# CasperTheCat/Vermilion

Measured on AMD Instinct MI355X. Metric: Mrays/sec (primary+secondary), 1920x1080 Sponza, higher is better.
Workload: dtype f32

## Files before the change

include/vermilion_hip.h:

```cpp
#ifndef VERMILION_HIP_H
#define VERMILION_HIP_H

#include <stdint.h>

#ifdef __cplusplus
extern "C" {
#endif

#define VMX_ABI_VERSION 2

#define VMX_OK 0
#define VMX_ERR_INVALID 1
#define VMX_ERR_NO_DEVICE 2
#define VMX_ERR_HIP 3
#define VMX_ERR_DEPTH 4
#define VMX_ERR_NOMEM 5

#define VMX_SPHERE_EMIT 1u

#define VMX_SAMPLING_PARITY 0u
#define VMX_SAMPLING_CORRECTED 1u
#define VMX_SAMPLING_MODE_MASK 0xFFu
#define VMX_SAMPLING_LIBM_DOUBLE 0x100u
#define VMX_SAMPLING_ELIDE_DEAD 0x200u
// ... 146 lines not shown
int vmx_query_device(const vmx_scene *scene, uint32_t mode, const void *d_origin, const void *d_dir,
                     const void *d_tmax, uint32_t n, void *d_tri_id, void *d_t, void *d_hit, void *stream);
int vmx_query(const vmx_scene *scene, uint32_t mode, const float *origin, const float *dir, const float *tmax,
              uint32_t n, int32_t *tri_id, float *t, uint8_t *hit);
int vmx_raycast_device(const vmx_scene *scene, const void *d_origin, const void *d_dir, uint32_t n, void *d_out,
                       uint32_t flags, void *stream);
int vmx_raycast_camera_device(const vmx_scene *scene, const vmx_camera *cam, const vmx_opts *opts, uint32_t k,
                              void *d_out, uint32_t flags, void *stream);

int vmx_primary_ids(const vmx_scene *scene, const vmx_camera *cam, const vmx_opts *opts, uint32_t k,
                    int32_t *tri_id, float *t);

int vmx_pixel_claims(const vmx_scene *scene, const vmx_camera *cam, const vmx_opts *opts, uint32_t *claims_out,
                     uint32_t *n_claimed);
int vmx_fused_camera_paths(const vmx_scene *scene, uint64_t *paths);
int vmx_pixel_claim_lists(const vmx_scene *scene, const vmx_camera *cam, const vmx_opts *opts, uint32_t *claims_out,
                          uint32_t *lists_out, uint32_t *n_claimed);
int vmx_list_settled_rays(const vmx_scene *scene, uint64_t *rays);
int vmx_guide_rays(const vmx_scene *scene, uint64_t *settled, uint64_t *fallback);
int vmx_guide_list_entries(const vmx_scene *scene, uint64_t *entries);
int vmx_guide_fused_rays(const vmx_scene *scene, uint64_t *settled, uint64_t *fallback);
int vmx_guide_trace(const vmx_scene *scene, const float *origin, const float *dir, uint32_t n, const vmx_opts *opts,
                    uint32_t flags, uint32_t grid_blocks, uint8_t *settled, uint32_t *slot, float *t);
int vmx_guide_trace_visits(const vmx_scene *scene, const float *origin, const float *dir, uint32_t n, const vmx_opts *opts,
                           uint32_t flags, uint32_t grid_blocks, uint8_t *settled, uint32_t *slot, float *t,
                           uint32_t *inner_visits, uint32_t *tri_tests);
int vmx_radiance(const vmx_scene *scene, const float *origin, const float *dir, uint32_t n,
                 const vmx_opts *opts, float *out, vmx_stats *stats);

int vmx_trig(const float *x, uint32_t n, float *cos_out, float *sin_out, int device);
// ... 252 lines not shown
```

vermilion_amd/_lib.py:

```python
import ctypes as C
import os

_HERE = os.path.dirname(os.path.abspath(__file__))
LIB_PATH = os.environ.get("VMX_LIB") or os.path.join(_HERE, "libvermilion_hip.so")

VMX_OK = 0
VMX_ERR_INVALID = 1
VMX_ERR_NO_DEVICE = 2
VMX_ERR_HIP = 3
VMX_ERR_DEPTH = 4
VMX_ERR_NOMEM = 5

VMX_SPHERE_EMIT = 1
VMX_SAMPLING_PARITY = 0
VMX_SAMPLING_CORRECTED = 1
VMX_SAMPLING_LIBM_DOUBLE = 0x100
VMX_SAMPLING_ELIDE_DEAD = 0x200
VMX_BVH_REFERENCE = 0
VMX_BVH_SAH = 1
VMX_BVH_LBVH = 2
VMX_BVH_PLOC = 3
VMX_BF_ABS_INT = 1
VMX_ROTATION_DEGREES = 0
VMX_ROTATION_RADIANS = 1
# ... 274 lines not shown
    "vmx_scene_compute_units": (C.c_uint32, [_P]),
    "vmx_scene_bvh": (C.c_int, [_P, _P, _P, _P, _P, _P]),
    "vmx_scene_update": (C.c_int, [_P, _P, _P, _P, C.c_uint32, C.c_uint32]),
    "vmx_scene_update_device": (C.c_int, [_P, _P, _P, _P, C.c_uint32, C.c_uint32, _P]),
    "vmx_scene_set_spheres": (C.c_int, [_P, _P, C.c_uint32]),
    "vmx_trace": (C.c_int, [_P, _P, _P, C.c_uint32, _P, _P]),
    "vmx_raycast": (C.c_int, [_P, _P, _P, C.c_uint32, _P]),
    "vmx_query_device": (C.c_int, [_P, C.c_uint32, _P, _P, _P, C.c_uint32, _P, _P, _P, _P]),
    "vmx_query": (C.c_int, [_P, C.c_uint32, _P, _P, _P, C.c_uint32, _P, _P, _P]),
    "vmx_raycast_device": (C.c_int, [_P, _P, _P, C.c_uint32, _P, C.c_uint32, _P]),
    "vmx_raycast_camera_device": (C.c_int, [_P, C.POINTER(CameraDesc), C.POINTER(Opts), C.c_uint32, _P, C.c_uint32,
                                            _P]),
    "vmx_primary_ids": (C.c_int, [_P, C.POINTER(CameraDesc), C.POINTER(Opts), C.c_uint32, _P, _P]),
    "vmx_pixel_claims": (C.c_int, [_P, C.POINTER(CameraDesc), C.POINTER(Opts), _P, C.POINTER(C.c_uint32)]),
    "vmx_fused_camera_paths": (C.c_int, [_P, C.POINTER(C.c_uint64)]),
    "vmx_pixel_claim_lists": (C.c_int, [_P, C.POINTER(CameraDesc), C.POINTER(Opts), _P, _P, C.POINTER(C.c_uint32)]),
    "vmx_list_settled_rays": (C.c_int, [_P, C.POINTER(C.c_uint64)]),
    "vmx_guide_rays": (C.c_int, [_P, C.POINTER(C.c_uint64), C.POINTER(C.c_uint64)]),
    "vmx_guide_list_entries": (C.c_int, [_P, C.POINTER(C.c_uint64)]),
    "vmx_guide_fused_rays": (C.c_int, [_P, C.POINTER(C.c_uint64), C.POINTER(C.c_uint64)]),
    "vmx_guide_trace": (C.c_int, [_P, _P, _P, C.c_uint32, _P, C.c_uint32, C.c_uint32, _P, _P, _P]),
    "vmx_guide_trace_visits": (C.c_int, [_P, _P, _P, C.c_uint32, _P, C.c_uint32, C.c_uint32, _P, _P, _P, _P, _P]),
    "vmx_radiance": (C.c_int, [_P, _P, _P, C.c_uint32, C.POINTER(Opts), _P, C.POINTER(Stats)]),
    "vmx_trig": (C.c_int, [_P, C.c_uint32, _P, _P, C.c_int]),
    "vmx_local_rows": (C.c_int, [C.c_uint32, C.c_uint32, C.c_uint32, C.c_uint32, C.POINTER(C.c_uint32)]),
    "vmx_render": (C.c_int, [_P, C.POINTER(CameraDesc), C.POINTER(Opts), _P, C.POINTER(Stats)]),
    "vmx_render_device": (C.c_int, [_P, C.POINTER(CameraDesc), C.POINTER(Opts), _P, _P, C.POINTER(Stats)]),
    "vmx_progressive_begin": (C.c_int, [_P, C.POINTER(CameraDesc), C.POINTER(Opts), _P, C.POINTER(_P)]),
    "vmx_progressive_step": (C.c_int, [_P, C.c_uint32, C.POINTER(Stats)]),
    "vmx_progressive_info_get": (C.c_int, [_P, C.POINTER(ProgressiveInfo)]),
# ... 125 lines not shown
```

vermilion_amd/csrc/api_claims.inc:

```
namespace {

constexpr uint32_t kClaimMinSamples = 64;
uint32_t claim_min_samples() {
#ifdef VMX_AB_KERNELS
    if (const char *e = std::getenv("VMX_CLAIM_MIN_SPP")) {
        const unsigned long v = std::strtoul(e, nullptr, 10);
        if (v) return (uint32_t)std::min<unsigned long>(v, 0xFFFFFFFFul);
    }
#endif
    return kClaimMinSamples;
}

int build_claims(vmx_scene *sc, const FrameDev &fr, const Tuning &tn, uint32_t npix, bool lists, hipStream_t s) {
    Workspace &ws = sc->ws;
    if (ws.claims.ensure((size_t)npix + 2)) return fail(VMX_ERR_NOMEM, "hipMalloc failed for the pixel claims");
    if (lists && ws.claim_lists.ensure((size_t)npix * kListWords)) return fail(VMX_ERR_NOMEM, "hipMalloc failed for the claim lists");
    WorkDev wk = make_work(nullptr, nullptr);
    wk.cam_inner = ws.cam_inner.p, wk.cam_tris = ws.cam_inner.p + std::max<size_t>(sc->n_inner, 1) * 64 * 8;
    const uint64_t tiles = (uint64_t)((fr.width + 7u) / 8u) * ((fr.local_rows + 7u) / 8u);
    if (tiles * 64 > 0xFFFFFFFFull) return fail(VMX_ERR_INVALID, "frame too large for the pixel claims");
    int cblocks = 0;
    HIP_TRY((hipError_t)query_pixel_claims_blocks_per_cu(kPathsBlock, (kPathsBlock / 64) * (tn.lds_primary + 1) * 512, &cblocks));
    if (cblocks < 1) return fail(VMX_ERR_HIP, "kernel does not fit on a CU (LDS stack too deep?)");
    LaunchCfg cfg = paths_cfg(sc, tn.lds_primary, tiles * 64, cblocks);
// ... 70 lines not shown
    vmx_scene *sc = const_cast<vmx_scene *>(csc);
    if (!sc || !rays) return fail(VMX_ERR_INVALID, "NULL argument");
    std::lock_guard<std::mutex> lock(sc->mu);
    *rays = sc->list_settled;
    return VMX_OK;
}

int vmx_fused_camera_paths(const vmx_scene *csc, uint64_t *paths) {
    vmx_scene *sc = const_cast<vmx_scene *>(csc);
    if (!sc || !paths) return fail(VMX_ERR_INVALID, "NULL argument");
    std::lock_guard<std::mutex> lock(sc->mu);
    *paths = sc->fused_paths;
    return VMX_OK;
}

}
```

vermilion_amd/csrc/api_render.inc:

```
namespace {

int nee_launch_cfg(vmx_scene *sc, hipStream_t s, const Tuning &tn, uint64_t items, bool rays, WorkDev &wk, LaunchCfg &cfg,
                   bool budgeted = false);

Tuning make_tuning(const vmx_scene *sc, const vmx_opts *o) {
    Tuning tn;
    tn.refill_min = o->reserved[3] ? o->reserved[3] : 8u;
    tn.refill_primary = o->reserved[3] ? o->reserved[3] : 64u;
    tn.shade_min = o->reserved[4] ? o->reserved[4] : 16u;
    tn.leaf_min = 0xFFFFFFFFu;
    tn.sort_mode = o->reserved[5];
    const uint32_t cap = o->reserved[6];
    tn.lds_entries = std::min(sc->dev.stack_entries, cap ? cap : 10u);
    tn.lds_primary = std::min(sc->dev.stack_entries, cap ? cap : (uint32_t)VMX_LDS_PRIMARY);
    tn.lds_bounce = std::min(sc->dev.stack_entries, cap ? cap : 9u);
    tn.tail_threshold = o->reserved[2] ? o->reserved[2] : (16u << 20);
    return tn;
}


int bind_stack(vmx_scene *sc, const Tuning &tn, uint32_t entries, uint32_t grid, uint64_t items, WorkDev &wk, bool guided) {
    const uint64_t per_lane = items / ((uint64_t)grid * kPathsBlock);
    wk.reserve = per_lane >= 256 ? 256u : (per_lane >= 64 ? 128u : 64u);
    wk.lds_entries = entries;
// ... 137 lines not shown
    DevCounters h;
    HIP_TRY(hipMemcpy(&h, ws.counters.p, sizeof(h), hipMemcpyDeviceToHost));
    if (h.overflow) return fail(VMX_ERR_NOMEM, "path queue overflow (sub-queues full); lower max paths per pass");
    vmx_stats local_stats;
    if (!stats) stats = &local_stats;
    std::memset(stats, 0, sizeof(*stats));
    stage_out(stats->primary, h.stage[0]);
    stage_out(stats->bounce, h.stage[1]);
    stats->rays_primary = h.stage[0].rays;
    stats->rays_secondary = h.stage[1].rays;
    stats->samples = h.samples;
    stats->samples_discarded = h.discarded;
    stats->passes = passes;
    stats->kernel_launches = launches;
    sc->fused_paths = h.fused;
    sc->list_settled = h.listed;
    unsigned long long guide_rays[2] = {0, 0};
    if (ws.guide_ctr.p) HIP_TRY(hipMemcpy(guide_rays, ws.guide_ctr.p, sizeof(guide_rays), hipMemcpyDeviceToHost));
    sc->guide_settled = guide_rays[0], sc->guide_fallback = guide_rays[1];
    unsigned long long fused_rays[2] = {0, 0};
    if (ws.guide_fused_ctr.p) HIP_TRY(hipMemcpy(fused_rays, ws.guide_fused_ctr.p, sizeof(fused_rays), hipMemcpyDeviceToHost));
    sc->guide_fused_settled = fused_rays[0], sc->guide_fused_fallback = fused_rays[1];
    sc->guide_entries = ws.guide_entries, ws.guide_entries = 0;
    std::memset(&sc->timings, 0, sizeof(sc->timings));
    for (auto &tl : timed) {
        float ms = 0.f;
        HIP_TRY(hipEventElapsedTime(&ms, tl.a, tl.b));
        if (tl.stage >= 0) {
            vmx_stage_stats &st = tl.stage == 0 ? stats->primary : (tl.stage == 1 ? stats->bounce : stats->shade);
            st.ms += ms;
// ... 15 lines not shown
    const uint32_t bits = opts->reserved[0];
    Forms f;
    f.pipeline = bits & kFormPipeline;
    f.count = opts->collect_counters != 0;
    f.split_any = f.pipeline == 0 || f.pipeline == 4;
    f.legacy = f.pipeline >= 2 && f.pipeline <= 3;
    f.two_phase = !f.count && !(bits & kFormOnePhase) && fr.r2scale == 10.0f;
    f.sorted = f.two_phase && !(bits & kFormKeepEnds);
    f.pool = ab_pool_bit(opts) && !f.sorted && !f.count;
    f.guide = sc->guide.valid && !f.count && !ab_pool_bit(opts) && !(bits & kFormNoGuide);
    f.bounce_records = f.split_any && !f.two_phase && !f.count && !f.pool && fr.r2scale == 10.0f;
    f.elide = f.split_any && fr.elide_dead;
    f.claims_on = f.split_any && !f.count && !f.elide && !(bits & kFormNoClaims);
    f.fuse_on = f.claims_on && !f.two_phase && !f.sorted && !(bits & kFormNoFuse);
    f.lists_on = f.claims_on && !(bits & kFormNoLists);
    return f;
}

int render_setup(vmx_scene *sc, const vmx_camera *cam, const vmx_opts *opts, PixelBufs *pixels, float *d_out, hipStream_t s,
                 RenderJob &job) {
    FrameDev &fr = job.fr;
    int rc = make_frame(*cam, *opts, fr);
    if (rc) return rc;
    job.opts = *opts;
    job.pixels = pixels, job.d_out = d_out, job.s = s;
    Workspace &ws = sc->ws;
    const uint32_t W = fr.width, rows = fr.local_rows;
    const uint32_t npix = job.npix = W * rows;
    if (opts->collect_counters) fr.elide_dead = 0;
    if ((opts->reserved[0] & kFormPipeline) > 4 || (opts->reserved[0] & ~kFormsRender)) return fail(VMX_ERR_INVALID, "unknown pipeline form");
// ... 300 lines not shown
    } else {
        LAUNCH_TRY(launch_shade(sc->dev, fr, wk, job.px, job.pa, qi[0], 0, ws.counters.p, false, (uint32_t)sc->num_cus, s));
    }
    return timed_end(job.timed, s);
}

int pass_split(vmx_scene *sc, RenderJob &job, WorkDev &wk) {
    Workspace &ws = sc->ws;
    const Tuning &tn = job.tn;
    hipStream_t s = job.s;
    const uint64_t items = (uint64_t)wk.n_pad * wk.samples;
    wk.refill_min = tn.refill_primary;
    wk.cam_inner = ws.cam_inner.p, wk.cam_tris = ws.cam_inner.p + std::max<size_t>(sc->n_inner, 1) * 64 * 8;
    wk.cam_n_inner = sc->n_inner;
    wk.claims = job.claims;
    wk.claim_lists = job.f.elide ? nullptr : job.claim_lists, wk.list_ctr = ws.counters.p;
    LaunchCfg cfg = paths_cfg(sc, tn.lds_primary, items, job.tb);
    int rc = bind_stack(sc, tn, tn.lds_primary, cfg.grid, items, wk);
    if (rc) return rc;
    HIP_TRY(hipMemsetAsync(ws.heads.p, 0, kSubQueues * 32 * 4, s));
    SplitRoute r;
    if ((rc = split_raygen(sc, job, wk, r))) return rc;
    if ((rc = split_trace(sc, job, wk, r, cfg))) return rc;
    if ((rc = split_shade(sc, job, wk, r))) return rc;
    job.launches += 4;
    return run_ids(sc, job.fr, job.pa, job.qi, 0, ws.counters.p, job.f, tn, s, job.timed, job.launches, job.tbb, job.rb);
}

int render_pass(vmx_scene *sc, RenderJob &job, uint32_t cap, uint32_t *taken) {
    Workspace &ws = sc->ws;
// ... 124 lines not shown
```

vermilion_amd/csrc/vmx_device.h:

```cpp
#pragma once
#include <stdint.h>

namespace vmx {

constexpr uint32_t kLeafBit = 0x80000000u;
constexpr uint32_t kLeafStartMask = 0x03FFFFFFu;
constexpr uint32_t kLeafCountShift = 26;
constexpr uint32_t kMaxLeafSize = 31;
constexpr uint32_t kMaxTris = kLeafStartMask + 1;
constexpr uint32_t kMaxSpheres = 16;
constexpr uint32_t kMaxStack = 64;

struct InnerRecord {
    float lmin[3];
    float lmax[3];
    float rmin[3];
    float rmax[3];
    uint32_t left, right, pad0, pad1;
};
static_assert(sizeof(InnerRecord) == 64, "inner record must be 64 bytes");

struct TriRecord {
    float v0[3];
    float e1[3];
// ... 32 lines not shown
    uint32_t tex_w, tex_h, tex_c;
    uint32_t tri_off;
    const float *tex1;
    uint32_t tex1_w, tex1_h, tex1_c;
    uint32_t emit_prefix;
};

struct StageCounters {
    unsigned long long rays, inner_visits, tri_tests, tri_hits, continued;
};
struct DevCounters {
    StageCounters stage[2];
    unsigned long long samples, discarded, pixels_done, overflow;
    unsigned long long fused;
    unsigned long long listed;
};

struct FastDiv {
    uint32_t m, sh1, sh2, d;
};
inline FastDiv make_fastdiv(uint32_t d) {
    if (d == 0) d = 1;
    uint32_t l = 0;
    while ((1ull << l) < d) ++l;
    FastDiv f;
    f.m = (uint32_t)((((1ull << l) - d) << 32) / d + 1ull);
    f.sh1 = l < 1 ? l : 1u;
    f.sh2 = l > 0 ? l - 1 : 0u;
    f.d = d;
    return f;
// ... 29 lines not shown
```

vermilion_amd/csrc/vmx_host.h:

```cpp
namespace {

thread_local std::string g_err;

int fail(int code, const std::string &msg) {
    g_err = msg;
    return code;
}

#define HIP_TRY(expr)                                                                              \
    do {                                                                                           \
        hipError_t e_ = (expr);                                                                    \
        if (e_ != hipSuccess)                                                                      \
            return fail(VMX_ERR_HIP, std::string(#expr) + ": " + hipGetErrorString(e_));           \
    } while (0)

#define LAUNCH_TRY(expr)                                                                           \
    do {                                                                                           \
        int e_ = (expr);                                                                           \
        if (e_ != 0)                                                                               \
            return fail(VMX_ERR_HIP, std::string(#expr) + ": " + hipGetErrorString((hipError_t)e_)); \
    } while (0)

const vmx_sphere kReferenceSpheres[8] = {
    {{15.f, 140.f, 25.f}, 3.5f, {0.f * 15.f, .5f * 15.f, 1.0f * 15.f}, VMX_SPHERE_EMIT, {-55.f, 350.f, -150.f}, -1.f},
// ... 156 lines not shown
    bool flat_topology = true;
    uint32_t n_inner = 0;
    uint32_t ntris = 0, leaf_size = 4;
    std::vector<vmx_sphere> spheres;
    DevBuf<unsigned char> d_geom;
    DevBuf<AttrRecord> d_attrs;
    DevBuf<SphereDev> d_spheres;
    DevBuf<float> d_tex, d_tex1;
    uint32_t n_textures = 0;
    SceneDev dev{};
    std::mutex mu;
    Workspace ws;
    uint32_t block = 256;
    float bounds_lo[3] = {0, 0, 0}, bounds_hi[3] = {1, 1, 1};
    vmx_timings timings{};
    uint64_t fused_paths = 0;
    uint64_t list_settled = 0;
    uint64_t guide_settled = 0, guide_fallback = 0;
    uint64_t guide_entries = 0;
    uint64_t guide_fused_settled = 0, guide_fused_fallback = 0;
    struct VMX_OPAQUE Guide {
        std::shared_ptr<const HostBvh> host;
        const unsigned char *base = nullptr;
        uint32_t off = 0;
        size_t bytes = 0;
        uint32_t tri_off = 0, root_ref = 0, stack_entries = 0;
        float scene_max = 0.f;
        bool valid = false;
    } guide;
    struct QueryWs {
// ... 226 lines not shown
    WorkDev wk;
    std::memset(&wk, 0, sizeof(wk));
    wk.heads = heads;
    if (tn) wk.refill_min = tn->refill_min, wk.shade_min = tn->shade_min;
    return wk;
}

constexpr uint32_t kFormPipeline = 0xFFu;
constexpr uint32_t kFormOnePhase = 1u << 8;
constexpr uint32_t kFormKeepEnds = 1u << 9;
constexpr uint32_t kFormPool = 1u << 10;
constexpr uint32_t kFormNoClaims = 1u << 11;
constexpr uint32_t kFormNoFuse = 1u << 12;
constexpr uint32_t kFormNoLists = 1u << 13;
constexpr uint32_t kFormNoGuide = 1u << 14;
constexpr uint32_t kFormsRender = kFormPipeline | kFormOnePhase | kFormKeepEnds | kFormPool | kFormNoClaims | kFormNoFuse | kFormNoLists | kFormNoGuide;
constexpr uint32_t kFormsRadiance = kFormPipeline | kFormOnePhase | kFormKeepEnds | kFormPool;

struct Forms {
    uint32_t pipeline = 0;
    bool count = false;
    bool split_any = false, legacy = false;
    bool two_phase = false;
    bool sorted = false;
    bool pool = false;
    bool guide = false;
    bool bounce_records = false;
    bool elide = false;
    bool claims_on = false;
    bool fuse_on = false;
    bool lists_on = false;
};

constexpr uint32_t kPathsBlock = 256;

struct RenderJob {
    FrameDev fr;
    vmx_opts opts;
    Tuning tn;
    Forms f;
    uint32_t npix = 0;
    bool nee = false;
    uint32_t smax = 0, smax_alloc = 0;
    uint32_t n_pad_max = 0, sub_cap = 0;
    uint64_t mem_budget = 0;
    int pb = 1, bb = 1, rb = 1, tb = 1, tbb = 1;
// ... 22 lines not shown
```

vermilion_amd/csrc/vmx_kernels.h:

```cpp
#pragma once
#include <stdint.h>
#include "vmx_device.h"

namespace vmx {

constexpr uint32_t kSubQueues = 16;

struct QueueDev {
    void *planes;
    unsigned int *counts;
    uint32_t capacity;
    uint32_t sub_capacity;
};

struct PixelStateDev {
    void *accum;
    unsigned int *count;
    unsigned int *cursor;
};

struct PathArrays {
    void *rayA;
    void *state;
    void *hit;
// ... 37 lines not shown
    uint32_t pool_slots;
    uint32_t out_capacity;
    const unsigned int *flat_ids;
    const unsigned int *flat_count;
    const void *cam_inner;
    uint32_t cam_n_inner;
    const void *cam_tris;
    const unsigned int *claims;
    const unsigned int *claim_lists;
    DevCounters *list_ctr;
    const unsigned int *unclaimed;
    const unsigned int *unclaimed_count;
    const unsigned int *shade_slots;
    const unsigned int *shade_count;
    uint32_t fused;
};

struct GuideDev {
    const void *base;
    uint32_t tri_off, root_ref;
    float scene_max;
    uint32_t fb_capacity;
    unsigned int *fb_ids;
    unsigned int *fb_count;
    unsigned long long *ctr;
    DevCounters *overflow;
};

struct GuidePathsDev {
    uint32_t off;
    uint32_t tri_off;
// ... 270 lines not shown
```

vermilion_amd/csrc/vmx_kernels.hip:

```cpp
#include <hip/hip_runtime.h>
#include <math.h>
#include <algorithm>
#include <stdint.h>

#include "vmx_kernels.h"
#include "pixel_claim.h"
#include "guide_walk.h"
#include <type_traits>

#ifndef VMX_CAM_BATCH
#define VMX_CAM_BATCH 16
#endif
#ifndef VMX_TRACE_WAVES_PER_SIMD
#define VMX_TRACE_WAVES_PER_SIMD 7
#endif


namespace vmx {
__device__ __forceinline__ float luminance(float r, float g, float b);
namespace {

constexpr float kInf = __builtin_huge_valf();

struct Cnt {
// ... 716 lines not shown
        (void)rng_next(P.rng);
        (void)rng_next(P.rng);
        (void)rng_next(P.rng);
        m.angle = r1;
        m.q = (float)sqrt(1.0 - r2);
    }
    if (m.q != m.q) return kPathEnded;
    return kPathNeedsTrig;
}

__device__ __forceinline__ bool path_shade_end(Path &P, const CastResult &c, StepFlags &fl, const ShadeMid &m, float cs,
                                               float sn) {
    const bool facing = dot3(c.nx, c.ny, c.nz, P.dx, P.dy, P.dz) < 0.f;
    const float wx = facing ? c.nx : c.nx * -1.f, wy = facing ? c.ny : c.ny * -1.f,
                wz = facing ? c.nz : c.nz * -1.f;
    const bool use_y = (double)fabsf(wx) > .1;
    const float ax = use_y ? 0.f : 1.f, ay = use_y ? 1.f : 0.f, az = 0.f;
    float ux, uy, uz, vx, vy, vz;
    cross3(ax, ay, az, wx, wy, wz, ux, uy, uz);
    normalize3(ux, uy, uz);
    cross3(wx, wy, wz, ux, uy, uz, vx, vy, vz);
    float ndx = (ux * cs * m.r2s + vx * sn * m.r2s) + wx * m.q;
    float ndy = (uy * cs * m.r2s + vy * sn * m.r2s) + wy * m.q;
    float ndz = (uz * cs * m.r2s + vz * sn * m.r2s) + wz * m.q;
    normalize3(ndx, ndy, ndz);
    return path_set_ray(P, fl, m.sx, m.sy, m.sz, ndx, ndy, ndz);
}

template <bool TEX>
__device__ __forceinline__ uint32_t step_bits(const SceneDev &sc, float r2scale, Rng rng, uint32_t depth, float ox, float oy,
// ... 1334 lines not shown
#else
#define VMX_PROF_STEP(EX, OC) step(EX, OC)
#endif

constexpr uint32_t kOutChunk = 256;
#define VMX_TRACE_W_VISITS 0
#include "vmx_trace_w.inc"
#undef VMX_TRACE_W_VISITS
#define VMX_TRACE_W_VISITS 1
#include "vmx_trace_w.inc"
#undef VMX_TRACE_W_VISITS

#ifndef VMX_SHADE_WPS
#define VMX_SHADE_WPS 7
#endif
template <int SRC, bool TEX, bool ELIDE = false, int FROMQ = 0, bool DENSE = false, bool CLAIMED = false>
__global__ void __launch_bounds__(256, VMX_SHADE_WPS)
k_shade(SceneDev sc, FrameDev fr, WorkDev wk, PixelStateDev px, PathArrays pa, IdQueue qout, uint32_t max_chunks,
        DevCounters *ctr) {
    const float2 *__restrict__ hits = (const float2 *)pa.hit;
    float4 *__restrict__ rad = (float4 *)pa.rad;
    __shared__ float4 s_geom[kLdsSpheres];
    __shared__ float4 s_cam_op[kLdsSpheres];
    __shared__ float s_lmax[4][kLdsSpheres + 1];
    __shared__ uint32_t s_pix[4][6];
    if (threadIdx.x < min(sc.nspheres, kLdsSpheres)) {
        const SphereDev &q = sc.spheres[threadIdx.x];
        s_geom[threadIdx.x] = make_float4(q.cx, q.cy, q.cz, q.rad2);
        const float opx = q.cx - fr.px, opy = q.cy - fr.py, opz = q.cz - fr.pz;
        s_cam_op[threadIdx.x] = make_float4(opx, opy, opz, dot3(opx, opy, opz, opx, opy, opz));
    }
    __syncthreads();
    Tally tl = {{0, 0}, {0, 0}, {0, 0}};
    uint32_t items = (SRC == 0 ? (wk.samples * wk.n_pad + blockDim.x - 1) / blockDim.x : max_chunks * kSubQueues);
    uint32_t flat_n = 0;
    if (FROMQ == 1) flat_n = *wk.flat_count, items = (flat_n + blockDim.x - 1) / blockDim.x;
    if (FROMQ == 2) flat_n = min(*wk.out_count, wk.out_capacity), items = (flat_n + blockDim.x - 1) / blockDim.x;
    constexpr bool listed = SRC == 0 && ELIDE;
    uint32_t live_n = 0;
    if (listed) {
        live_n = *wk.live_count;
        if (FROMQ == 0) items = (live_n + blockDim.x - 1) / blockDim.x;
    }
    static_assert(!DENSE || (SRC == 0 && FROMQ == 0 && !ELIDE), "the dense form is the plain camera pass");
    static_assert(!CLAIMED || DENSE, "claimed pixels are fused in the dense form only");
    constexpr bool dense = DENSE;
    const uint32_t lane = threadIdx.x & 63u;
    const uint32_t wave = (uint32_t)__builtin_amdgcn_readfirstlane((int)(threadIdx.x >> 6));
    const uint32_t chunks = dense ? wk.samples >> 6 : 1u;
    uint32_t n_fused = 0;
    uint32_t unit = blockIdx.x, unit_step = gridDim.x, units = items;
    if (dense) {
        unit = (uint32_t)__builtin_amdgcn_readfirstlane((int)(blockIdx.x * (blockDim.x >> 6) + (threadIdx.x >> 6)));
        unit_step = gridDim.x * (blockDim.x >> 6), units = wk.shade_slots ? *wk.shade_count : wk.n_pad;
    }
    for (; unit < units; unit += unit_step) {
        const uint32_t slot = DENSE ? (wk.shade_slots ? wk.shade_slots[unit] : unit) : unit;
        const bool px_active = dense && slot < wk.n_active;
        uint32_t px_claim = kClaimNone, px_pixel = 0;
        if (px_active) {
            const uint32_t lp = wk.active[slot];
            const uint32_t pixel = global_pixel(fr, lp);
            if (CLAIMED) px_claim = wk.claims[lp], px_pixel = pixel;
            const PixelKey pk = rng_pixel_key(fr.seed, pixel);
            const uint32_t cur = px.cursor[lp];
// ... 39 lines not shown
                    if (listed) live_n = 0xFFFFFFFFu;
                }
                if (listed) pid = src < live_n ? wk.live_ids[src] : 0xFFFFFFFFu;
                uint32_t pixel = 0, k = 0, pid2;
                if (dense) {
                    const uint32_t j = ch * 64u + lane;
                    if (px_active) k = (fr.lead != 0 && j >= fr.lead) ? (j - fr.lead + 1u) * fr.quarter : s_pix[wave][0] + j * s_pix[wave][1];
                    run = px_active && k < fr.kmax;
                } else {
                    uint32_t j, s_idx;
                    if (wk.pixel_major) s_idx = fast_div(pid, wk.div_samples), j = pid - s_idx * wk.samples;
                    else j = pid / wk.n_pad, s_idx = pid - j * wk.n_pad;
                    run = j < wk.samples && s_idx < wk.n_pad && primary_item(fr, wk, px, j, s_idx, pid2, pixel, k);
                }
                if (CLAIMED) {
                    n_fused += (uint32_t)__popcll(__builtin_amdgcn_ballot_w64(run));
                    if (run) {
                        PixelKey pk;
                        pk.a = (uint64_t)s_pix[wave][2] | ((uint64_t)s_pix[wave][3] << 32);
                        pk.b = (uint64_t)s_pix[wave][4] | ((uint64_t)s_pix[wave][5] << 32);
                        P.ox = fr.px, P.oy = fr.py, P.oz = fr.pz, P.depth = 0;
                        primary_ray_keyed(fr, px_pixel, pk, k, P.rng, P.dx, P.dy, P.dz);
                        float best = 999999999.f;
                        int leaf = -1;
                        if (px_claim < kClaimMiss) {
                            typedef float f32x4 __attribute__((ext_vector_type(4)));
                            typedef const __attribute__((address_space(4))) f32x4 *scalar_ptr;
                            const uint32_t claim = (uint32_t)__builtin_amdgcn_readfirstlane((int)px_claim);
                            const scalar_ptr rec = (scalar_ptr)((uintptr_t)wk.cam_tris + (size_t)claim * 64u);
                            const f32x4 r0 = rec[0], r1 = rec[1], r2 = rec[2], r3 = rec[3];
                            float dist;
// ... 63 lines not shown
                    touch = P.depth == 0 || c.cr != 0.f || c.cg != 0.f || c.cb != 0.f;
                    if (TEX) touch = touch || !(finite3(P.tr, P.tg, P.tb) && fabsf(P.tw) < kInf);
                    if (touch) {
                        had = rad_has(pa, pid);
                        const float4 acc = rad_fetch(pa, pid, had);
                        P.ar = acc.x, P.ag = acc.y, P.ab = acc.z, P.aw = acc.w;
                    }
                }
                st = path_shade_begin<TEX>(sc, fr.r2scale, P, c, fl, mid);
                if (SRC != 0) {
                    if (touch) rad_commit(pa, pid, make_float4(P.ar, P.ag, P.ab, P.aw), had);
                } else if (!pa.rad_mask) {
                    rad[pid] = make_float4(P.ar, P.ag, P.ab, P.aw);
                }
            }
            bool alive = st == kPathNextRay;
            if (st == kPathNeedsTrig) {
                float sn, cs;
                shade_trig(mid, fr.libm_double, cs, sn);
                alive = path_shade_end(P, c, fl, mid, cs, sn);
            }
            if (ELIDE && alive &&
                step_is_dead<TEX>(sc, fr.r2scale, P.rng, P.depth, P.ox, P.oy, P.oz, P.dx, P.dy, P.dz, P.tr, P.tg, P.tb))
                alive = false, fl.continues = false;
            if (alive) {
                uint32_t bits = 0;
                if (fr.bounce_bits) bits = step_bits<TEX>(sc, fr.r2scale, P.rng, P.depth, P.ox, P.oy, P.oz, P.dx, P.dy, P.dz, P.tr, P.tg, P.tb);
                ray_store(pa, pid, P, bits);
                rng_store(pa, pid, P.rng);
                if (TEX) ((float4 *)pa.thr)[pid] = make_float4(P.tr, P.tg, P.tb, P.tw);
            }
            if (SRC == 0 && pa.rad_mask) {
                const bool need = run && (P.ar != 0.f || P.ag != 0.f || P.ab != 0.f);
                if (need) rad[pid] = make_float4(P.ar, P.ag, P.ab, P.aw);
                if (listed || FROMQ != 0) {
                    if (need) atomicOr(&pa.rad_mask[pid >> 6], 1ull << (pid & 63u));
                } else {
                    const unsigned long long word = __builtin_amdgcn_ballot_w64(need);
                    if (lane == 0) pa.rad_mask[pos0 >> 6] = word;
                }
            }
            tally_add(tl, fl, run, depth0);
            id_append(qout, item % kSubQueues, alive, pid);
        }
    }
    const Cnt none = {0, 0};
    tally_flush<false>(ctr, tl, none, none);
    if (CLAIMED && lane == 0 && n_fused) atomicAdd(&ctr->fused, (unsigned long long)n_fused);
}

template <int SRC, bool TEX, bool LISTED>
__global__ void __launch_bounds__(256)
k_shade_ends(SceneDev sc, FrameDev fr, WorkDev wk, PathArrays pa, unsigned long long *__restrict__ full_mask,
             unsigned int *__restrict__ full_cnt, uint32_t max_chunks, DevCounters *ctr) {
    const float2 *__restrict__ hits = (const float2 *)pa.hit;
    float4 *__restrict__ rad = (float4 *)pa.rad;
    __shared__ float4 s_geom[kLdsSpheres];
    __shared__ float4 s_cam_op[kLdsSpheres];
    __shared__ float4 s_col[kLdsSpheres];
    const uint32_t nlight = min(sc.emit_prefix, kLdsSpheres);
    if (threadIdx.x < nlight) {
        const SphereDev &q = sc.spheres[threadIdx.x];
        s_geom[threadIdx.x] = make_float4(q.cx, q.cy, q.cz, q.rad2);
// ... 700 lines not shown
}

int query_trace_q_blocks_per_cu(uint32_t block, uint32_t lds_bytes, bool count, bool from_queue, bool sorted, bool live, int *blocks,
                                bool guide) {
    int a = 0;
    const hipError_t e = count ? hipOccupancyMaxActiveBlocksPerMultiprocessor(&a, trace_q_kernel(from_queue), (int)block, lds_bytes)
                               : hipOccupancyMaxActiveBlocksPerMultiprocessor(&a, trace_w_kernel(from_queue, sorted, live, guide && from_queue), (int)block, lds_bytes);
    if (blocks) *blocks = a;
    return (int)e;
}

int launch_shade(const SceneDev &sc, const FrameDev &fr, const WorkDev &wk, PixelStateDev px, PathArrays pa,
                 IdQueue qout, uint32_t max_chunks, DevCounters *counters, bool from_queue, uint32_t cus, void *stream) {
    hipStream_t s = (hipStream_t)stream;
    const bool flat = wk.flat_ids != nullptr || wk.out_rec != nullptr;
    const uint32_t shade_grid = std::max(cus, 1u) * VMX_SHADE_WPS;
    const bool dense = !from_queue && !flat && !wk.live_ids && wk.pixel_major && (wk.samples & 63u) == 0;
    const uint64_t items = flat ? shade_grid
                                : (from_queue ? (uint64_t)max_chunks * kSubQueues
                                              : (dense ? ((uint64_t)wk.n_pad + 3) / 4 : ((uint64_t)wk.samples * wk.n_pad + 255) / 256));
    uint32_t grid = (uint32_t)std::min<uint64_t>(items, shade_grid);
    if (grid == 0) grid = 1;
#define VMX_GO(S, T, E, Q, D)                                                                                                    \
    do {                                  \
        if (D && wk.fused) hipLaunchKernelGGL((k_shade<S, T, E, Q, D, D>), dim3(grid), dim3(256), 0, s, sc, fr, wk, px, pa, qout, max_chunks, counters); \
        else hipLaunchKernelGGL((k_shade<S, T, E, Q, D>), dim3(grid), dim3(256), 0, s, sc, fr, wk, px, pa, qout, max_chunks, counters); \
    } while (0)
#define VMX_GO_T(S, E, Q, ...)                       \
    do {                                             \
        if (sc.tex) VMX_GO(S, true, E, Q, (false __VA_ARGS__)); \
        else VMX_GO(S, false, E, Q, (false __VA_ARGS__));     \
    } while (0)
// ... 136 lines not shown
```

vermilion_amd/scene.py:

```python
import ctypes as C

import numpy as np

from . import _lib as L


def _is_tensor(x):
    return type(x).__module__.startswith("torch") and hasattr(x, "data_ptr")


def _f32(a, shape_last=None):
    a = np.ascontiguousarray(a, dtype=np.float32)
    if shape_last is not None and (a.ndim == 0 or a.shape[-1] != shape_last):
        a = a.reshape(-1, shape_last)
    return a


def _device_rays(x, name):
    import torch
    if not _is_tensor(x):
        raise ValueError(f"{name}: mix of torch tensors and other arrays")
    if x.dim() != 2 or x.shape[1] != 3:
        raise ValueError(f"{name} must be [n, 3]")
    if x.dtype != torch.float32:
# ... 582 lines not shown
                                     C.byref(st)))
        return out, st.as_dict()

    def pixel_claims(self, cam, opts):
        rows = local_rows(cam.image_res[1], opts.stripe_rows, opts.rank, opts.world)
        out = np.empty((rows, cam.image_res[0]), np.uint32)
        n = C.c_uint32(0)
        self._check(self._lib.vmx_pixel_claims(self._h, C.byref(cam), C.byref(opts), out.ctypes.data, C.byref(n)))
        return out, int(n.value)

    def fused_camera_paths(self):
        n = C.c_uint64(0)
        self._check(self._lib.vmx_fused_camera_paths(self._h, C.byref(n)))
        return int(n.value)

    def pixel_claim_lists(self, cam, opts):
        rows = local_rows(cam.image_res[1], opts.stripe_rows, opts.rank, opts.world)
        out = np.empty((rows, cam.image_res[0]), np.uint32)
        lists = np.empty((rows, cam.image_res[0], 4), np.uint32)
        n = C.c_uint32(0)
        self._check(self._lib.vmx_pixel_claim_lists(self._h, C.byref(cam), C.byref(opts), out.ctypes.data, lists.ctypes.data,
                                                    C.byref(n)))
        return out, lists, int(n.value)

    def list_settled_rays(self):
        n = C.c_uint64(0)
        self._check(self._lib.vmx_list_settled_rays(self._h, C.byref(n)))
        return int(n.value)

    def guide_rays(self):
# ... 463 lines not shown
```

Measured before the change: 13280.

## Park surviving shade lanes in LDS and compact before continuation work

In the dense shade kernel, lanes whose paths continue are compacted into a per-wave shared-memory park. When enough have accumulated, they are reloaded densely so the lobe sampling, ray setup and queue append run with full wavefronts instead of sparse divergent ones. This adds LDS storage and occupancy pressure (launch bounds and grid reduced by one wave per SIMD for the textured variant), extra LDS traffic, and a replay path when the park would overflow. New counters and an API expose how many paths were parked, flushed and handled directly.

Result: slower. 11630 (-12.4%).

```diff
diff --git a/include/vermilion_hip.h b/include/vermilion_hip.h
--- a/include/vermilion_hip.h
+++ b/include/vermilion_hip.h
@@ -184,6 +184,7 @@
 int vmx_pixel_claims(const vmx_scene *scene, const vmx_camera *cam, const vmx_opts *opts, uint32_t *claims_out,
                      uint32_t *n_claimed);
 int vmx_fused_camera_paths(const vmx_scene *scene, uint64_t *paths);
+int vmx_shade_park_counts(const vmx_scene *scene, uint64_t *parked, uint64_t *flushes, uint64_t *direct);
 int vmx_pixel_claim_lists(const vmx_scene *scene, const vmx_camera *cam, const vmx_opts *opts, uint32_t *claims_out,
                           uint32_t *lists_out, uint32_t *n_claimed);
 int vmx_list_settled_rays(const vmx_scene *scene, uint64_t *rays);
diff --git a/vermilion_amd/_lib.py b/vermilion_amd/_lib.py
--- a/vermilion_amd/_lib.py
+++ b/vermilion_amd/_lib.py
@@ -312,6 +312,7 @@
     "vmx_primary_ids": (C.c_int, [_P, C.POINTER(CameraDesc), C.POINTER(Opts), C.c_uint32, _P, _P]),
     "vmx_pixel_claims": (C.c_int, [_P, C.POINTER(CameraDesc), C.POINTER(Opts), _P, C.POINTER(C.c_uint32)]),
     "vmx_fused_camera_paths": (C.c_int, [_P, C.POINTER(C.c_uint64)]),
+    "vmx_shade_park_counts": (C.c_int, [_P, C.POINTER(C.c_uint64), C.POINTER(C.c_uint64), C.POINTER(C.c_uint64)]),
     "vmx_pixel_claim_lists": (C.c_int, [_P, C.POINTER(CameraDesc), C.POINTER(Opts), _P, _P, C.POINTER(C.c_uint32)]),
     "vmx_list_settled_rays": (C.c_int, [_P, C.POINTER(C.c_uint64)]),
     "vmx_guide_rays": (C.c_int, [_P, C.POINTER(C.c_uint64), C.POINTER(C.c_uint64)]),
diff --git a/vermilion_amd/csrc/api_claims.inc b/vermilion_amd/csrc/api_claims.inc
--- a/vermilion_amd/csrc/api_claims.inc
+++ b/vermilion_amd/csrc/api_claims.inc
@@ -108,4 +108,12 @@
     return VMX_OK;
 }
 
+int vmx_shade_park_counts(const vmx_scene *csc, uint64_t *parked, uint64_t *flushes, uint64_t *direct) {
+    vmx_scene *sc = const_cast<vmx_scene *>(csc);
+    if (!sc || !parked || !flushes || !direct) return fail(VMX_ERR_INVALID, "NULL argument");
+    std::lock_guard<std::mutex> lock(sc->mu);
+    *parked = sc->park_counts[0], *flushes = sc->park_counts[1], *direct = sc->park_counts[2];
+    return VMX_OK;
 }
+
+}
diff --git a/vermilion_amd/csrc/api_render.inc b/vermilion_amd/csrc/api_render.inc
--- a/vermilion_amd/csrc/api_render.inc
+++ b/vermilion_amd/csrc/api_render.inc
@@ -175,6 +175,7 @@
     stats->passes = passes;
     stats->kernel_launches = launches;
     sc->fused_paths = h.fused;
+    sc->park_counts[0] = h.parked, sc->park_counts[1] = h.park_flushes, sc->park_counts[2] = h.park_direct;
     sc->list_settled = h.listed;
     unsigned long long guide_rays[2] = {0, 0};
     if (ws.guide_ctr.p) HIP_TRY(hipMemcpy(guide_rays, ws.guide_ctr.p, sizeof(guide_rays), hipMemcpyDeviceToHost));
@@ -220,6 +221,7 @@
     f.claims_on = f.split_any && !f.count && !f.elide && !(bits & kFormNoClaims);
     f.fuse_on = f.claims_on && !f.two_phase && !f.sorted && !(bits & kFormNoFuse);
     f.lists_on = f.claims_on && !(bits & kFormNoLists);
+    f.defer_on = f.split_any && !(bits & kFormNoDefer);
     return f;
 }
 
@@ -550,6 +552,7 @@
     wk.cam_inner = ws.cam_inner.p, wk.cam_tris = ws.cam_inner.p + std::max<size_t>(sc->n_inner, 1) * 64 * 8;
     wk.cam_n_inner = sc->n_inner;
     wk.claims = job.claims;
+    wk.defer_min = job.f.defer_on ? kDeferDirectMin : 0u;
     wk.claim_lists = job.f.elide ? nullptr : job.claim_lists, wk.list_ctr = ws.counters.p;
     LaunchCfg cfg = paths_cfg(sc, tn.lds_primary, items, job.tb);
     int rc = bind_stack(sc, tn, tn.lds_primary, cfg.grid, items, wk);
diff --git a/vermilion_amd/csrc/vmx_device.h b/vermilion_amd/csrc/vmx_device.h
--- a/vermilion_amd/csrc/vmx_device.h
+++ b/vermilion_amd/csrc/vmx_device.h
@@ -70,6 +70,7 @@
     unsigned long long samples, discarded, pixels_done, overflow;
     unsigned long long fused;
     unsigned long long listed;
+    unsigned long long parked, park_flushes, park_direct;
 };
 
 struct FastDiv {
diff --git a/vermilion_amd/csrc/vmx_host.h b/vermilion_amd/csrc/vmx_host.h
--- a/vermilion_amd/csrc/vmx_host.h
+++ b/vermilion_amd/csrc/vmx_host.h
@@ -194,6 +194,7 @@
     uint32_t block = 256;
     float bounds_lo[3] = {0, 0, 0}, bounds_hi[3] = {1, 1, 1};
     vmx_timings timings{};
+    uint64_t park_counts[3] = {0, 0, 0};
     uint64_t fused_paths = 0;
     uint64_t list_settled = 0;
     uint64_t guide_settled = 0, guide_fallback = 0;
@@ -450,7 +451,8 @@
 constexpr uint32_t kFormNoFuse = 1u << 12;
 constexpr uint32_t kFormNoLists = 1u << 13;
 constexpr uint32_t kFormNoGuide = 1u << 14;
-constexpr uint32_t kFormsRender = kFormPipeline | kFormOnePhase | kFormKeepEnds | kFormPool | kFormNoClaims | kFormNoFuse | kFormNoLists | kFormNoGuide;
+constexpr uint32_t kFormNoDefer = 1u << 15;
+constexpr uint32_t kFormsRender = kFormPipeline | kFormOnePhase | kFormKeepEnds | kFormPool | kFormNoClaims | kFormNoFuse | kFormNoLists | kFormNoGuide | kFormNoDefer;
 constexpr uint32_t kFormsRadiance = kFormPipeline | kFormOnePhase | kFormKeepEnds | kFormPool;
 
 struct Forms {
@@ -466,6 +468,7 @@
     bool claims_on = false;
     bool fuse_on = false;
     bool lists_on = false;
+    bool defer_on = false;
 };
 
 constexpr uint32_t kPathsBlock = 256;
diff --git a/vermilion_amd/csrc/vmx_kernels.h b/vermilion_amd/csrc/vmx_kernels.h
--- a/vermilion_amd/csrc/vmx_kernels.h
+++ b/vermilion_amd/csrc/vmx_kernels.h
@@ -5,6 +5,11 @@
 namespace vmx {
 
 constexpr uint32_t kSubQueues = 16;
+#ifndef VMX_DEFER_DIRECT_MIN
+#define VMX_DEFER_DIRECT_MIN 32
+#endif
+constexpr uint32_t kDeferDirectMin = VMX_DEFER_DIRECT_MIN;
+static_assert(kDeferDirectMin <= 64, "a parked chunk's lanes fit an empty park");
 
 struct QueueDev {
     void *planes;
@@ -75,7 +80,9 @@
     const unsigned int *shade_slots;
     const unsigned int *shade_count;
     uint32_t fused;
-};
+    uint32_t defer_min;
+};
+static_assert(sizeof(WorkDev) == 296, "WorkDev::defer_min lies in the former tail padding");
 
 struct GuideDev {
     const void *base;
diff --git a/vermilion_amd/csrc/vmx_kernels.hip b/vermilion_amd/csrc/vmx_kernels.hip
--- a/vermilion_amd/csrc/vmx_kernels.hip
+++ b/vermilion_amd/csrc/vmx_kernels.hip
@@ -754,6 +754,24 @@
     const bool facing = dot3(c.nx, c.ny, c.nz, P.dx, P.dy, P.dz) < 0.f;
     const float wx = facing ? c.nx : c.nx * -1.f, wy = facing ? c.ny : c.ny * -1.f,
                 wz = facing ? c.nz : c.nz * -1.f;
+    const bool use_y = (double)fabsf(wx) > .1;
+    const float ax = use_y ? 0.f : 1.f, ay = use_y ? 1.f : 0.f, az = 0.f;
+    float ux, uy, uz, vx, vy, vz;
+    cross3(ax, ay, az, wx, wy, wz, ux, uy, uz);
+    normalize3(ux, uy, uz);
+    cross3(wx, wy, wz, ux, uy, uz, vx, vy, vz);
+    float ndx = (ux * cs * m.r2s + vx * sn * m.r2s) + wx * m.q;
+    float ndy = (uy * cs * m.r2s + vy * sn * m.r2s) + wy * m.q;
+    float ndz = (uz * cs * m.r2s + vz * sn * m.r2s) + wz * m.q;
+    normalize3(ndx, ndy, ndz);
+    return path_set_ray(P, fl, m.sx, m.sy, m.sz, ndx, ndy, ndz);
+}
+__device__ __forceinline__ void path_lobe_normal(const Path &P, const CastResult &c, float &wx, float &wy, float &wz) {
+    const bool facing = dot3(c.nx, c.ny, c.nz, P.dx, P.dy, P.dz) < 0.f;
+    wx = facing ? c.nx : c.nx * -1.f, wy = facing ? c.ny : c.ny * -1.f, wz = facing ? c.nz : c.nz * -1.f;
+}
+__device__ __forceinline__ bool path_lobe_ray(Path &P, StepFlags &fl, const ShadeMid &m, float wx, float wy, float wz, float cs,
+                                              float sn) {
     const bool use_y = (double)fabsf(wx) > .1;
     const float ax = use_y ? 0.f : 1.f, ay = use_y ? 1.f : 0.f, az = 0.f;
     float ux, uy, uz, vx, vy, vz;
@@ -2118,8 +2136,116 @@
 #ifndef VMX_SHADE_WPS
 #define VMX_SHADE_WPS 7
 #endif
+#ifndef VMX_PARK_FLUSH_AT
+#define VMX_PARK_FLUSH_AT 48
+#endif
+constexpr uint32_t kParkFlushAt = VMX_PARK_FLUSH_AT;
+constexpr uint32_t kParkRng = 0, kParkPid = 8, kParkOrg = 9, kParkDir = 12, kParkR2s = 15, kParkQ = 16, kParkAngleF = 17,
+                   kParkAngle = 18, kParkThr = 20;
+template <bool TEX>
+constexpr uint32_t kParkPlanes = TEX ? 24u : 20u;
+struct ParkEntry {
+    Rng rng;
+    uint32_t pid;
+    float sx, sy, sz, wx, wy, wz, r2s, q, angle_f;
+    double angle;
+    float tr, tg, tb, tw;
+};
+template <bool TEX>
+__device__ __forceinline__ void park_entry(ParkEntry &e, int st, const Path &P, const CastResult &c, const ShadeMid &m) {
+    e.wx = P.dx, e.wy = P.dy, e.wz = P.dz, e.q = __uint_as_float(0x7FC00000u);
+    if (st == kPathNeedsTrig) path_lobe_normal(P, c, e.wx, e.wy, e.wz), e.q = m.q;
+    e.rng = P.rng;
+    e.pid = P.dest;
+    e.sx = m.sx, e.sy = m.sy, e.sz = m.sz;
+    e.r2s = m.r2s, e.angle_f = m.angle_f, e.angle = m.angle;
+    e.tr = P.tr, e.tg = P.tg, e.tb = P.tb, e.tw = P.tw;
+}
+template <bool TEX>
+__device__ __forceinline__ void park_store(uint32_t *park, uint32_t at, const ParkEntry &e) {
+    const uint64_t a = (uint64_t)__double_as_longlong(e.angle);
+    park[(kParkRng + 0) * 64 + at] = (uint32_t)e.rng.s0, park[(kParkRng + 1) * 64 + at] = (uint32_t)(e.rng.s0 >> 32);
+    park[(kParkRng + 2) * 64 + at] = (uint32_t)e.rng.s1, park[(kParkRng + 3) * 64 + at] = (uint32_t)(e.rng.s1 >> 32);
+    park[(kParkRng + 4) * 64 + at] = (uint32_t)e.rng.s2, park[(kParkRng + 5) * 64 + at] = (uint32_t)(e.rng.s2 >> 32);
+    park[(kParkRng + 6) * 64 + at] = (uint32_t)e.rng.s3, park[(kParkRng + 7) * 64 + at] = (uint32_t)(e.rng.s3 >> 32);
+    park[kParkPid * 64 + at] = e.pid;
+    park[(kParkOrg + 0) * 64 + at] = __float_as_uint(e.sx), park[(kParkOrg + 1) * 64 + at] = __float_as_uint(e.sy);
+    park[(kParkOrg + 2) * 64 + at] = __float_as_uint(e.sz);
+    park[(kParkDir + 0) * 64 + at] = __float_as_uint(e.wx), park[(kParkDir + 1) * 64 + at] = __float_as_uint(e.wy);
+    park[(kParkDir + 2) * 64 + at] = __float_as_uint(e.wz);
+    park[kParkR2s * 64 + at] = __float_as_uint(e.r2s), park[kParkQ * 64 + at] = __float_as_uint(e.q);
+    park[kParkAngleF * 64 + at] = __float_as_uint(e.angle_f);
+    park[kParkAngle * 64 + at] = (uint32_t)a, park[(kParkAngle + 1) * 64 + at] = (uint32_t)(a >> 32);
+    if (TEX) {
+        park[(kParkThr + 0) * 64 + at] = __float_as_uint(e.tr), park[(kParkThr + 1) * 64 + at] = __float_as_uint(e.tg);
+        park[(kParkThr + 2) * 64 + at] = __float_as_uint(e.tb), park[(kParkThr + 3) * 64 + at] = __float_as_uint(e.tw);
+    }
+}
+template <bool TEX>
+__device__ __forceinline__ void park_load(const uint32_t *park, uint32_t at, ParkEntry &e) {
+    e.rng.s0 = (uint64_t)park[(kParkRng + 0) * 64 + at] | ((uint64_t)park[(kParkRng + 1) * 64 + at] << 32);
+    e.rng.s1 = (uint64_t)park[(kParkRng + 2) * 64 + at] | ((uint64_t)park[(kParkRng + 3) * 64 + at] << 32);
+    e.rng.s2 = (uint64_t)park[(kParkRng + 4) * 64 + at] | ((uint64_t)park[(kParkRng + 5) * 64 + at] << 32);
+    e.rng.s3 = (uint64_t)park[(kParkRng + 6) * 64 + at] | ((uint64_t)park[(kParkRng + 7) * 64 + at] << 32);
+    e.pid = park[kParkPid * 64 + at];
+    e.sx = __uint_as_float(park[(kParkOrg + 0) * 64 + at]), e.sy = __uint_as_float(park[(kParkOrg + 1) * 64 + at]);
+    e.sz = __uint_as_float(park[(kParkOrg + 2) * 64 + at]);
+    e.wx = __uint_as_float(park[(kParkDir + 0) * 64 + at]), e.wy = __uint_as_float(park[(kParkDir + 1) * 64 + at]);
+    e.wz = __uint_as_float(park[(kParkDir + 2) * 64 + at]);
+    e.r2s = __uint_as_float(park[kParkR2s * 64 + at]), e.q = __uint_as_float(park[kParkQ * 64 + at]);
+    e.angle_f = __uint_as_float(park[kParkAngleF * 64 + at]);
+    e.angle = __longlong_as_double((long long)((uint64_t)park[kParkAngle * 64 + at] | ((uint64_t)park[(kParkAngle + 1) * 64 + at] << 32)));
+    if (TEX) {
+        e.tr = __uint_as_float(park[(kParkThr + 0) * 64 + at]), e.tg = __uint_as_float(park[(kParkThr + 1) * 64 + at]);
+        e.tb = __uint_as_float(park[(kParkThr + 2) * 64 + at]), e.tw = __uint_as_float(park[(kParkThr + 3) * 64 + at]);
+    }
+}
+
+template <bool TEX>
+__device__ __forceinline__ void park_finish(const ParkEntry &e, bool have, const SceneDev &sc, const FrameDev &fr,
+                                            const PathArrays &pa, const IdQueue &qout, Tally &tl) {
+    bool alive = false;
+    uint32_t pid = 0;
+    StepFlags fl = {false, false, false};
+    if (have) {
+        Path P;
+        ShadeMid m;
+        P.rng = e.rng;
+        P.dest = pid = e.pid;
+        P.depth = 1;
+        m.sx = e.sx, m.sy = e.sy, m.sz = e.sz;
+        const float wx = e.wx, wy = e.wy, wz = e.wz;
+        m.r2s = e.r2s, m.q = e.q, m.angle_f = e.angle_f, m.angle = e.angle;
+        P.tr = P.tg = P.tb = P.tw = 1.f;
+        if (TEX) P.tr = e.tr, P.tg = e.tg, P.tb = e.tb, P.tw = e.tw;
+        if (m.q != m.q) {
+            alive = path_set_ray(P, fl, m.sx, m.sy, m.sz, wx, wy, wz);
+        } else {
+            float sn, cs;
+            shade_trig(m, fr.libm_double, cs, sn);
+            alive = path_lobe_ray(P, fl, m, wx, wy, wz, cs, sn);
+        }
+        if (alive) {
+            uint32_t bits = 0;
+            if (fr.bounce_bits) bits = step_bits<TEX>(sc, fr.r2scale, P.rng, P.depth, P.ox, P.oy, P.oz, P.dx, P.dy, P.dz, P.tr, P.tg, P.tb);
+            ray_store(pa, pid, P, bits);
+            rng_store(pa, pid, P.rng);
+            if (TEX) ((float4 *)pa.thr)[pid] = make_float4(P.tr, P.tg, P.tb, P.tw);
+        }
+    }
+    tl.cont[0] += (uint32_t)__popcll(__ballot(fl.continues));
+    const uint32_t sub = (pid >> 8) % kSubQueues;
+    unsigned long long rest = __ballot(alive);
+    while (rest) {
+        const uint32_t s = (uint32_t)__builtin_amdgcn_readlane((int)sub, __ffsll((long long)rest) - 1);
+        const bool mine = alive && sub == s;
+        id_append(qout, s, mine, pid);
+        rest &= ~__ballot(mine);
+    }
+}
+
 template <int SRC, bool TEX, bool ELIDE = false, int FROMQ = 0, bool DENSE = false, bool CLAIMED = false>
-__global__ void __launch_bounds__(256, VMX_SHADE_WPS)
+__global__ void __launch_bounds__(256, (DENSE && TEX) ? VMX_SHADE_WPS - 1 : VMX_SHADE_WPS)
 k_shade(SceneDev sc, FrameDev fr, WorkDev wk, PixelStateDev px, PathArrays pa, IdQueue qout, uint32_t max_chunks,
         DevCounters *ctr) {
     const float2 *__restrict__ hits = (const float2 *)pa.hit;
@@ -2128,6 +2254,7 @@
     __shared__ float4 s_cam_op[kLdsSpheres];
     __shared__ float s_lmax[4][kLdsSpheres + 1];
     __shared__ uint32_t s_pix[4][6];
+    __shared__ uint32_t s_park[DENSE ? 4 : 1][DENSE ? kParkPlanes<TEX> * 64 : 1];
     if (threadIdx.x < min(sc.nspheres, kLdsSpheres)) {
         const SphereDev &q = sc.spheres[threadIdx.x];
         s_geom[threadIdx.x] = make_float4(q.cx, q.cy, q.cz, q.rad2);
@@ -2153,6 +2280,7 @@
     const uint32_t wave = (uint32_t)__builtin_amdgcn_readfirstlane((int)(threadIdx.x >> 6));
     const uint32_t chunks = dense ? wk.samples >> 6 : 1u;
     uint32_t n_fused = 0;
+    uint32_t pending = 0, n_parked = 0, n_flushes = 0, n_direct = 0;
     uint32_t unit = blockIdx.x, unit_step = gridDim.x, units = items;
     if (dense) {
         unit = (uint32_t)__builtin_amdgcn_readfirstlane((int)(blockIdx.x * (blockDim.x >> 6) + (threadIdx.x >> 6)));
@@ -2222,7 +2350,6 @@
                     run = j < wk.samples && s_idx < wk.n_pad && primary_item(fr, wk, px, j, s_idx, pid2, pixel, k);
                 }
                 if (CLAIMED) {
-                    n_fused += (uint32_t)__popcll(__builtin_amdgcn_ballot_w64(run));
                     if (run) {
                         PixelKey pk;
                         pk.a = (uint64_t)s_pix[wave][2] | ((uint64_t)s_pix[wave][3] << 32);
@@ -2316,8 +2443,32 @@
                     rad[pid] = make_float4(P.ar, P.ag, P.ab, P.aw);
                 }
             }
-            bool alive = st == kPathNextRay;
-            if (st == kPathNeedsTrig) {
+            bool alive = !DENSE && st == kPathNextRay;
+            const bool lobe = !DENSE && st == kPathNeedsTrig;
+            bool redo = false, flush = false;
+            if (DENSE) {
+                const unsigned long long go = __builtin_amdgcn_ballot_w64(st != kPathEnded);
+                const uint32_t n = (uint32_t)__popcll(go);
+                if (n != 0) {
+                    if (pending + n > 64u) {
+                        redo = true;
+                    } else {
+                        if (st != kPathEnded) {
+                            ParkEntry entry;
+                            park_entry<TEX>(entry, st, P, c, mid);
+                            park_store<TEX>(s_park[wave], pending + (uint32_t)__popcll(go & ((1ull << lane) - 1ull)), entry);
+                        }
+                        __builtin_amdgcn_fence(__ATOMIC_RELEASE, "wavefront");
+                        __builtin_amdgcn_wave_barrier();
+                        pending += n;
+                        flush = n >= wk.defer_min;
+                        if (!flush) n_parked += n;
+                        else if (wk.defer_min) n_direct += n;
+                    }
+                }
+                fl.continues = false;
+            }
+            if (lobe) {
                 float sn, cs;
                 shade_trig(mid, fr.libm_double, cs, sn);
                 alive = path_shade_end(P, c, fl, mid, cs, sn);
@@ -2342,13 +2493,31 @@
                     if (lane == 0) pa.rad_mask[pos0 >> 6] = word;
                 }
             }
-            tally_add(tl, fl, run, depth0);
-            id_append(qout, item % kSubQueues, alive, pid);
+            if (!redo) tally_add(tl, fl, run, depth0);
+            if (CLAIMED && !redo) n_fused += (uint32_t)__popcll(__builtin_amdgcn_ballot_w64(run));
+            if (!DENSE) id_append(qout, item % kSubQueues, alive, pid);
+            if (DENSE) {
+                if (pending != 0 && (redo || flush || pending > kParkFlushAt || (ch + 1 == chunks && unit + unit_step >= units))) {
+                    ParkEntry entry;
+                    if (lane < pending) park_load<TEX>(s_park[wave], lane, entry);
+                    __builtin_amdgcn_fence(__ATOMIC_RELEASE, "wavefront");
+                    __builtin_amdgcn_wave_barrier();
+                    park_finish<TEX>(entry, lane < pending, sc, fr, pa, qout, tl);
+                    pending = 0;
+                    if (wk.defer_min) n_flushes++;
+                }
+                if (redo) --ch;
+            }
         }
     }
     const Cnt none = {0, 0};
     tally_flush<false>(ctr, tl, none, none);
     if (CLAIMED && lane == 0 && n_fused) atomicAdd(&ctr->fused, (unsigned long long)n_fused);
+    if (DENSE && lane == 0) {
+        if (n_parked) atomicAdd(&ctr->parked, (unsigned long long)n_parked);
+        if (n_flushes) atomicAdd(&ctr->park_flushes, (unsigned long long)n_flushes);
+        if (n_direct) atomicAdd(&ctr->park_direct, (unsigned long long)n_direct);
+    }
 }
 
 template <int SRC, bool TEX, bool LISTED>
@@ -3079,8 +3248,8 @@
                  IdQueue qout, uint32_t max_chunks, DevCounters *counters, bool from_queue, uint32_t cus, void *stream) {
     hipStream_t s = (hipStream_t)stream;
     const bool flat = wk.flat_ids != nullptr || wk.out_rec != nullptr;
-    const uint32_t shade_grid = std::max(cus, 1u) * VMX_SHADE_WPS;
     const bool dense = !from_queue && !flat && !wk.live_ids && wk.pixel_major && (wk.samples & 63u) == 0;
+    const uint32_t shade_grid = std::max(cus, 1u) * (dense && sc.tex ? VMX_SHADE_WPS - 1 : VMX_SHADE_WPS);
     const uint64_t items = flat ? shade_grid
                                 : (from_queue ? (uint64_t)max_chunks * kSubQueues
                                               : (dense ? ((uint64_t)wk.n_pad + 3) / 4 : ((uint64_t)wk.samples * wk.n_pad + 255) / 256));
diff --git a/vermilion_amd/scene.py b/vermilion_amd/scene.py
--- a/vermilion_amd/scene.py
+++ b/vermilion_amd/scene.py
@@ -620,6 +620,11 @@
         self._check(self._lib.vmx_fused_camera_paths(self._h, C.byref(n)))
         return int(n.value)
 
+    def shade_park_counts(self):
+        p, f, d = C.c_uint64(0), C.c_uint64(0), C.c_uint64(0)
+        self._check(self._lib.vmx_shade_park_counts(self._h, C.byref(p), C.byref(f), C.byref(d)))
+        return int(p.value), int(f.value), int(d.value)
+
     def pixel_claim_lists(self, cam, opts):
         rows = local_rows(cam.image_res[1], opts.stripe_rows, opts.rank, opts.world)
         out = np.empty((rows, cam.image_res[0]), np.uint32)
```
